# GeoStat-Framework/PyKrige

Hardware: NVIDIA H100
Metric: kriged grid points/sec (N data -> M grid) (higher is better)
Workload: dtype f64

## Files before the change

### pykrige_b200/csrc/api.cu

```cuda
#include <cuda_runtime.h>
#include <string>
#include <vector>
#include <cstring>
#include <cstdio>
#include <cmath>
#include <cstdlib>
#include <algorithm>
#include <thread>
#include <climits>
#include "kernels.h"

#define KB_VERSION 2000
static const int64_t KB_STAGE_PTS = 1 << 20;
#define KB_TILE_COST_32 0.607
#define KB_TILE_COST_16 0.403
static const int64_t KB_STAGE_MIN = 1 << 18;
#define KB_TN_FIELDS 32

struct Src {
    bool grid; int64_t nx, ny, nz;
    const double *a, *b, *c;
    int64_t first, count;
    const double* d_drift; int64_t drift_stride, drift_first;

    Src sub(int64_t o, int64_t m) const {
        Src s = *this; s.first += o; s.count = m; s.drift_first += o; return s;
    }
    PointSource point_source() const {
        PointSource ps{};
        ps.grid = grid ? 1 : 0;
        ps.px = a; ps.py = b; ps.pz = c; ps.gx = a; ps.gy = b; ps.gz = c;
        ps.nx = nx; ps.ny = ny; ps.nz = nz; ps.first = first;
        return ps;
    }
};

enum Tm { TM_ASSEMBLE, TM_CHOLESKY, TM_TRTRI, TM_PACK_DUAL, TM_SOLVE, TM_FINALIZE, TM_H2D, TM_D2H, TM_KNN_SEARCH,
          TM_KNN_SOLVE, TM_SOLVE_LAUNCHES, TM_LAUNCHES, TM_COUNT };
enum Ev { EV_UPLOAD, EV_ADJUSTED, EV_ASM, EV_KNN_BUILT = EV_ASM, EV_FACTOR, EV_INVERT, EV_DUAL, EV_PACKED,
          EV_RUN, EV_RUN_END, EV_H2D, EV_H2D_END, EV_D2H_END, EV_COUNT };

struct DevBuf {
    void* p = nullptr; size_t cap = 0;
    cudaError_t reserve(size_t bytes) {
        if (bytes <= cap) return cudaSuccess;
        if (p) cudaFree(p);
        p = nullptr; cap = 0;
        cudaError_t e = cudaMalloc(&p, bytes);
        if (e == cudaSuccess) cap = bytes;
        return e;
    }
    void release() { if (p) cudaFree(p); p = nullptr; cap = 0; }
    template <typename T> T* as() const { return reinterpret_cast<T*>(p); }
};

struct kb200_ctx {
    int device = 0;
    cudaStream_t stream = nullptr;
    bool own_stream = false;
    std::string err;

    bool described = false, ready = false, knn_ready = false;
    bool local_factor = false;
    int slices = 0;
    int gform = 0;
    int geo = 0;
    int pinv = 0;
    int pinv_sweeps = 0, pinv_rank = 0;
    int dim = 2, dtype = KB200_F64, n = 0, n_pad = 0, ld = 0, n_rl = 0, n_hd = 0, K1 = 1, na = 2, nrb = 0;
    VgParams vg{};
    Aniso an{};
    DriftScale ds{};
    PackMap pm{};
    std::vector<double> hx, hy, hz, hval, hdrift;
    double bb_lo[3] = {0, 0, 0}, bb_hi[3] = {0, 0, 0};
    int nf = 0; int64_t nf_n = 0;
    std::vector<double> hfields;
    int aux_cols = KB_MAXAUX;
    int64_t zstride = 0;
    int pin_blocks = 0;

    DevBuf blob;
    size_t off_consts = 0, off_ax = 0, off_ay = 0, off_az = 0, off_tiles = 0, off_rowscale = 0, blob_bytes = 0;

    DevBuf wC, wW, wT, wF, wRaw, wFlag;
    DevBuf wPts, wOut, wDrift, wScratch, wFstage;
    int num_sms = 132;
    DeviceDrift dd{};
    DevBuf wWells, wExt;
    int n_dev = 0;
    void* pin[2] = {nullptr, nullptr};
    cudaStream_t copy_stream = nullptr;
    cudaEvent_t evk[2] = {}, evc[2] = {};
    cudaStream_t hi_stream = nullptr;
    std::vector<cudaEvent_t> fev;
    DevBuf kSorted, kCells, kFields;
    DevBuf wVario;
    DevBuf wLoo;
    DevBuf wLgo, wLgoM;
    DevBuf wPairs;
    DevBuf wTab;
    std::vector<double> htab;
    double tab_dmax = 0.0; int tab_n = 0;
    KnnParams kp{};
    int k_ncells = 0;

    cudaEvent_t ev[EV_COUNT] = {};
    double tm[TM_COUNT] = {};
    long long launches = 0, solve_launches = 0;
};

static int fail(kb200_ctx* h, int code, const std::string& msg) {
    if (h) h->err = msg;
    return code;
}
#define CU(h, expr) do { cudaError_t _e = (expr); if (_e != cudaSuccess) { \
    return fail(h, _e == cudaErrorMemoryAllocation ? KB200_ENOMEM : KB200_ECUDA, \
                std::string(#expr) + ": " + cudaGetErrorString(_e)); } } while (0)

static size_t align_up(size_t v, size_t a) { return (v + a - 1) / a * a; }

static void drop_problem(kb200_ctx* h) {
    h->described = false; h->ready = false; h->knn_ready = false; h->local_factor = false;
}

struct BlobView { double *hdr, *consts, *ax, *ay, *az; char* tiles; double* rowscale; };
static BlobView blob_view(const kb200_ctx* h) {
    char* p = h->blob.as<char>();
    auto at = [p](size_t off) { return reinterpret_cast<double*>(p + off); };
    return {at(0), at(h->off_consts), at(h->off_ax), at(h->off_ay), at(h->off_az), p + h->off_tiles, at(h->off_rowscale)};
}

enum HdrSlot { HDR_MAGIC = 0, HDR_C0 = 1, HDR_SHIFT = 2, HDR_SCALE = HDR_SHIFT + KB200_MAX_DRIFT + 1,
               HDR_GFORM = HDR_SCALE + KB200_MAX_DRIFT + 1, HDR_DOUBLES = 64 };
static_assert(HDR_GFORM == 34 && HDR_GFORM < HDR_DOUBLES, "blob header layout");
static const double KB_MAGIC = 20260922.0;

static void write_header(const kb200_ctx* h, double* hdr) {
    std::fill(hdr, hdr + HDR_DOUBLES, 0.0);
    hdr[HDR_MAGIC] = KB_MAGIC; hdr[HDR_C0] = h->vg.c0; hdr[HDR_GFORM] = (double)h->gform;
    for (int c = 0; c <= KB200_MAX_DRIFT; ++c) { hdr[HDR_SHIFT + c] = h->ds.shift[c]; hdr[HDR_SCALE + c] = h->ds.scale[c]; }
}

static bool read_header(kb200_ctx* h, const double* hdr) {
    if (hdr[HDR_MAGIC] != KB_MAGIC) return false;
    h->vg.c0 = hdr[HDR_C0];
    h->gform = (int)hdr[HDR_GFORM];
    for (int c = 0; c <= KB200_MAX_DRIFT; ++c) { h->ds.shift[c] = hdr[HDR_SHIFT + c]; h->ds.scale[c] = hdr[HDR_SCALE + c]; }
    return true;
}

enum RawCol { RAW_X, RAW_Y, RAW_Z, RAW_V, RAW_DRIFT };
static double* raw_col(const kb200_ctx* h, int c) { return h->wRaw.as<double>() + (size_t)c * h->n; }
static double* kriged_values(const kb200_ctx* h) { return raw_col(h, h->nf ? RAW_DRIFT + h->n_hd : RAW_V); }

enum AuxBlock { AUX_F, AUX_H, AUX_U };
static double* aux_block(const kb200_ctx* h, int i) {
    return h->wF.as<double>() + (size_t)i * h->aux_cols * h->n_pad;
}

extern "C" int kb200_version(void) { return KB_VERSION; }

extern "C" int kb200_create(kb200_handle* out, int device) {
    if (!out) return KB200_EBADARG;
    *out = nullptr;
    int cnt = 0;
    cudaError_t e = cudaGetDeviceCount(&cnt);
    if (e != cudaSuccess || cnt == 0) return KB200_ECUDA;
    kb200_ctx* h = new kb200_ctx();
    if (device < 0) { if (cudaGetDevice(&device) != cudaSuccess) device = 0; }
    if (device >= cnt) { delete h; return KB200_EBADARG; }
    h->device = device;
    if (cudaSetDevice(device) != cudaSuccess) { delete h; return KB200_ECUDA; }
    if (cudaStreamCreateWithFlags(&h->stream, cudaStreamNonBlocking) != cudaSuccess) { delete h; return KB200_ECUDA; }
    h->own_stream = true;
    for (auto& ev : h->ev) if (cudaEventCreate(&ev) != cudaSuccess) { delete h; return KB200_ECUDA; }
    if (kbk_factor_init() != cudaSuccess || kbk_solve_init() != cudaSuccess || kbk_solve_tf32_init() != cudaSuccess ||
        kbk_solve_i8_init() != cudaSuccess || kbk_ev_init() != cudaSuccess || kbk_pinv_init() != cudaSuccess) { delete h; return KB200_ECUDA; }
    if (cudaDeviceGetAttribute(&h->num_sms, cudaDevAttrMultiProcessorCount, device) != cudaSuccess || h->num_sms < 1) h->num_sms = 132;
    *out = h;
    return KB200_OK;
}

extern "C" void kb200_destroy(kb200_handle h) {
    if (!h) return;
    cudaSetDevice(h->device);
    cudaStreamSynchronize(h->stream);
    for (DevBuf* b : {&h->blob, &h->wC, &h->wW, &h->wT, &h->wF, &h->wRaw, &h->wFlag,
                      &h->wPts, &h->wOut, &h->wDrift, &h->wScratch, &h->wFstage, &h->kSorted, &h->kCells, &h->kFields, &h->wVario, &h->wTab,
                      &h->wLoo, &h->wLgo, &h->wLgoM, &h->wPairs, &h->wWells, &h->wExt}) b->release();
    for (int i = 0; i < 2; ++i) {
        if (h->pin[i]) cudaFreeHost(h->pin[i]);
        if (h->evk[i]) cudaEventDestroy(h->evk[i]);
        if (h->evc[i]) cudaEventDestroy(h->evc[i]);
    }
    if (h->copy_stream) cudaStreamDestroy(h->copy_stream);
    if (h->hi_stream) cudaStreamDestroy(h->hi_stream);
    for (auto& e : h->fev) cudaEventDestroy(e);
    for (auto& ev : h->ev) if (ev) cudaEventDestroy(ev);
    if (h->own_stream && h->stream) cudaStreamDestroy(h->stream);
    delete h;
}

extern "C" const char* kb200_last_error(kb200_handle h) { return h ? h->err.c_str() : "null handle"; }

extern "C" int kb200_set_stream(kb200_handle h, void* s) {
    if (!h) return KB200_EBADARG;
    if (h->own_stream && h->stream) { cudaStreamSynchronize(h->stream); cudaStreamDestroy(h->stream); }
    h->stream = reinterpret_cast<cudaStream_t>(s);
    h->own_stream = false;
    return KB200_OK;
}

extern "C" int kb200_set_coordinates(kb200_handle h, int coordinates_type) {
    if (!h) return KB200_EBADARG;
    if (coordinates_type != KB200_EUCLIDEAN && coordinates_type != KB200_GEOGRAPHIC)
        return fail(h, KB200_EBADARG, "coordinates_type must be KB200_EUCLIDEAN or KB200_GEOGRAPHIC");
    h->geo = coordinates_type == KB200_GEOGRAPHIC ? 1 : 0;
    drop_problem(h);
    return KB200_OK;
}

extern "C" int kb200_set_pseudo_inverse(kb200_handle h, int enable) {
    if (!h) return KB200_EBADARG;
    h->pinv = enable ? 1 : 0;
    drop_problem(h);
    return KB200_OK;
}

extern "C" int kb200_set_values(kb200_handle h, int n_fields, int64_t n, const double* values) {
    if (!h) return KB200_EBADARG;
    drop_problem(h);
    h->nf = 0; h->nf_n = 0; h->hfields.clear();
    if (n_fields == 0) return KB200_OK;
    if (n_fields < 0 || n_fields > KB200_MAX_FIELDS)
        return fail(h, KB200_EBADARG, "n_fields must be in [0, " + std::to_string(KB200_MAX_FIELDS) + "]");
    if (n < 1 || n > (1LL << 30) || !values) return fail(h, KB200_EBADARG, "values: n >= 1 rows and a non-NULL array");
    const size_t cnt = (size_t)n * n_fields;
    for (size_t i = 0; i < cnt; ++i)
        if (!std::isfinite(values[i]))
            return fail(h, KB200_EBADARG, "values must be finite (field " + std::to_string(i / n) + ", row " +
                        std::to_string(i % n) + ")");
    h->hfields.assign(values, values + cnt);
    h->nf = n_fields; h->nf_n = n;
    return KB200_OK;
}

extern "C" void kb200_reset_counters(kb200_handle h) {
    if (!h) return;
    h->launches = 0; h->solve_launches = 0;
    for (double& t : h->tm) t = 0.0;
}

extern "C" int kb200_last_timings(kb200_handle h, double* ms, int n) {
    if (!h || !ms) return KB200_EBADARG;
    h->tm[TM_SOLVE_LAUNCHES] = (double)h->solve_launches;
    h->tm[TM_LAUNCHES] = (double)h->launches;
    int m = std::min(n, (int)TM_COUNT);
    for (int i = 0; i < m; ++i) ms[i] = h->tm[i];
    return m;
}

static double host_gamma(const kb200_ctx* h, const VgParams& v, double d) {
    switch (v.model) {
        case KB200_VG_LINEAR: return v.p0 * d + v.p1;
        case KB200_VG_POWER: return v.p0 * std::pow(d, v.p1) + v.p2;
        case KB200_VG_TABLE: {
            if (h->tab_n < 2) return 1.0;
            const double inv_h = (h->tab_n - 1) / std::sqrt(h->tab_dmax);
            int last = (int)std::min<double>(h->tab_n - 1, std::ceil(std::sqrt(std::max(d, 0.0)) * inv_h));
            double g = h->htab[0];
            for (int i = 0; i <= last; ++i) g = std::max(g, h->htab[2 * (size_t)i]);
            return g;
        }
        default: return v.p0 + v.p2;
    }
}

extern "C" int kb200_set_variogram_table(kb200_handle h, int64_t n_nodes, double dmax, const double* gamma_nodes) {
    if (!h) return KB200_EBADARG;
    if (n_nodes < 16 || n_nodes > (1LL << 26) || !gamma_nodes || !(dmax > 0.0) || !std::isfinite(dmax))
        return fail(h, KB200_EBADARG, "variogram table: 16 <= n_nodes <= 2^26, dmax > 0");
    const int n = (int)n_nodes;
    for (int i = 0; i < n; ++i)
        if (!std::isfinite(gamma_nodes[i])) return fail(h, KB200_EBADARG, "variogram table: the callable must be finite on [0, dmax] (node " + std::to_string(i) + ")");
    drop_problem(h);
    h->htab.resize(2 * (size_t)n);
    for (int i = 0; i < n; ++i) {
        double m;
        if (i == 0) m = -1.5 * gamma_nodes[0] + 2.0 * gamma_nodes[1] - 0.5 * gamma_nodes[2];
        else if (i == n - 1) m = 1.5 * gamma_nodes[n - 1] - 2.0 * gamma_nodes[n - 2] + 0.5 * gamma_nodes[n - 3];
        else m = 0.5 * (gamma_nodes[i + 1] - gamma_nodes[i - 1]);
        h->htab[2 * (size_t)i] = gamma_nodes[i];
        h->htab[2 * (size_t)i + 1] = m;
    }
    h->tab_n = n; h->tab_dmax = dmax;
    cudaSetDevice(h->device);
    CU(h, h->wTab.reserve(h->htab.size() * sizeof(double)));
    CU(h, cudaMemcpyAsync(h->wTab.p, h->htab.data(), h->htab.size() * sizeof(double), cudaMemcpyHostToDevice, h->stream));
    CU(h, cudaStreamSynchronize(h->stream));
    return KB200_OK;
}

static int describe(kb200_ctx* h, bool knn_only, int dim, int dtype, int64_t n,
                    const double* x, const double* y, const double* z, const double* values,
                    const double* center, const double* aniso, int model, const double* vparams, int n_vparams,
                    int exact_values, double eps, int n_rl, int n_hd, const double* drift_data) {
    if (!h) return KB200_EBADARG;
    drop_problem(h);
    if (dim != 2 && dim != 3) return fail(h, KB200_EBADARG, "dim must be 2 or 3");
    if (h->geo && dim != 2) return fail(h, KB200_EBADARG, "geographic coordinates are two-dimensional (lon, lat)");
    if (h->geo && (n_rl || n_hd)) return fail(h, KB200_EUNSUPPORTED, "universal kriging has no geographic mode (uk.py:337)");
    if (dtype < KB200_F64 || dtype > KB200_F64X4)
        return fail(h, KB200_EBADARG, "dtype must be KB200_F64, KB200_F32, KB200_F64X, KB200_F64X5 or KB200_F64X4");
    if (n < 1 || (!knn_only && n > (int64_t)(KB_MAXRB - 1) * KB_BM) || n > (1LL << 30)) return fail(h, KB200_EBADARG, "n out of range");
    if (!x || !y || (dim == 3 && !z) || !values || !center || !aniso || (!vparams && model != KB200_VG_TABLE))
        return fail(h, KB200_EBADARG, "null input array");
    if (model < KB200_VG_LINEAR || model > KB200_VG_TABLE)
// ... 1292 lines not shown
```

### pykrige_b200/csrc/common.cuh

```cuda
#pragma once
#include <cuda_runtime.h>
#include <stdint.h>
#include <math.h>
#include "../../include/krige_b200.h"

#define KB_WARP 32

#define KB_BM 256
#define KB_TN 64
#define KB_BK 16
#define KB_NB 64
#define KB_MAXAUX (KB200_MAX_DRIFT + 2)
#define KB_MAXRB 128

struct VgParams {
    int model;
    double p0, p1, p2;
    double inv_a;
    double c0;
    double eps;
    int exact;
    const double2* tab;
    double tab_inv_h;
    int tab_n;
};

struct Aniso {
    double m[9];
    double c[3];
};

#define KB_GEO 4
#define KB_HASZ(DIM) ((DIM) >= 3)

template <int DIM>
__device__ __forceinline__ void kb_adjust(const Aniso& a, double x, double y, double z,
                                          double& ox, double& oy, double& oz) {
    if (DIM == KB_GEO) {
        const double rad = 0.017453292519943295;
        double slon, clon, slat, clat;
        sincos(x * rad, &slon, &clon);
        sincos(y * rad, &slat, &clat);
        ox = clon * clat; oy = slon * clat; oz = slat;
        return;
    }
    double dx = __dsub_rn(x, a.c[0]);
    double dy = __dsub_rn(y, a.c[1]);
    if (DIM == 2) {
        double rx = __dadd_rn(__dmul_rn(a.m[0], dx), __dmul_rn(a.m[1], dy));
        double ry = __dadd_rn(__dmul_rn(a.m[2], dx), __dmul_rn(a.m[3], dy));
        ox = __dadd_rn(rx, a.c[0]);
        oy = __dadd_rn(ry, a.c[1]);
        oz = 0.0;
    } else {
        double dz = __dsub_rn(z, a.c[2]);
        double rx = __dadd_rn(__dadd_rn(__dmul_rn(a.m[0], dx), __dmul_rn(a.m[1], dy)), __dmul_rn(a.m[2], dz));
        double ry = __dadd_rn(__dadd_rn(__dmul_rn(a.m[3], dx), __dmul_rn(a.m[4], dy)), __dmul_rn(a.m[5], dz));
        double rz = __dadd_rn(__dadd_rn(__dmul_rn(a.m[6], dx), __dmul_rn(a.m[7], dy)), __dmul_rn(a.m[8], dz));
        ox = __dadd_rn(rx, a.c[0]);
        oy = __dadd_rn(ry, a.c[1]);
        oz = __dadd_rn(rz, a.c[2]);
    }
}

__device__ __forceinline__ double kb_exp_neg(double x) {
    const double kd = rint(x * 1.4426950408889634);
    double r = fma(kd, -6.93147180369123816490e-01, x);
    r = fma(kd, -1.90821492927058770002e-10, r);
    double p = 1.6059043836821613e-10;
    p = fma(p, r, 2.08767569878681e-09);
    p = fma(p, r, 2.505210838544172e-08);
    p = fma(p, r, 2.755731922398589e-07);
    p = fma(p, r, 2.7557319223985893e-06);
    p = fma(p, r, 2.48015873015873e-05);
    p = fma(p, r, 1.984126984126984e-04);
    p = fma(p, r, 1.388888888888889e-03);
    p = fma(p, r, 8.333333333333333e-03);
    p = fma(p, r, 4.1666666666666664e-02);
    p = fma(p, r, 1.6666666666666666e-01);
    p = fma(p, r, 0.5);
    p = fma(p, r, 1.0);
    p = fma(p, r, 1.0);
    const int k = (int)kd;
    const double v = __hiloint2double(__double2hiint(p) + (k << 20), __double2loint(p));
    return x < -708.0 ? 0.0 : v;
}

template <int MODEL>
__device__ __forceinline__ double kb_gamma(const VgParams& v, double d) {
    if (MODEL == KB200_VG_LINEAR) {
        return v.p0 * d + v.p1;
    } else if (MODEL == KB200_VG_POWER) {
        return v.p0 * pow(d, v.p1) + v.p2;
    } else if (MODEL == KB200_VG_GAUSSIAN) {
        return v.p0 * (1.0 - kb_exp_neg(-(d * d) * v.inv_a)) + v.p2;
    } else if (MODEL == KB200_VG_EXPONENTIAL) {
        return v.p0 * (1.0 - kb_exp_neg(-d * v.inv_a)) + v.p2;
    } else if (MODEL == KB200_VG_SPHERICAL) {
        if (d <= v.p1) {
            double q = d * v.inv_a;
            return v.p0 * (1.5 * q - 0.5 * q * q * q) + v.p2;
        }
        return v.p0 + v.p2;
    } else if (MODEL == KB200_VG_TABLE) {
        const double u = sqrt(d) * v.tab_inv_h;
        int i = (int)u;
        i = i > v.tab_n - 2 ? v.tab_n - 2 : i;
        const double t = u - (double)i;
        const double2 a = __ldg(v.tab + i), b = __ldg(v.tab + i + 1);
        const double t2 = t * t, t3 = t2 * t;
        return (2.0 * t3 - 3.0 * t2 + 1.0) * a.x + (t3 - 2.0 * t2 + t) * a.y
             + (3.0 * t2 - 2.0 * t3) * b.x + (t3 - t2) * b.y;
    } else {
        double q = d * v.inv_a;
        return v.p0 * (1.0 - (1.0 - q) * kb_exp_neg(-q)) + v.p2;
    }
}

template <int MODEL>
__device__ __forceinline__ double kb_cov_rhs(const VgParams& v, double d) {
    if (v.exact && fabs(d) <= v.eps) return v.c0;
    return v.c0 - kb_gamma<MODEL>(v, d);
}

template <int DIM>
__device__ __forceinline__ double kb_dist(double ax, double ay, double az,
                                          double bx, double by, double bz) {
    if (DIM == KB_GEO) {
        double cx = __dsub_rn(__dmul_rn(ay, bz), __dmul_rn(az, by));
        double cy = __dsub_rn(__dmul_rn(az, bx), __dmul_rn(ax, bz));
        double cz = __dsub_rn(__dmul_rn(ax, by), __dmul_rn(ay, bx));
        double s = sqrt(cx * cx + cy * cy + cz * cz);
        double c = ax * bx + ay * by + az * bz;
        return atan2(s, c) * 57.29577951308232;
    }
    double dx = ax - bx, dy = ay - by;
    double s = dx * dx + dy * dy;
    if (DIM == 3) { double dz = az - bz; s += dz * dz; }
    return sqrt(s);
}

struct PointSource {
    int grid;
    const double* px; const double* py; const double* pz;
    const double* gx; const double* gy; const double* gz;
    long long nx, ny, nz;
    long long first;
};

template <int DIM>
__device__ __forceinline__ void kb_load_point_raw(const PointSource& ps, long long p,
                                                  double& rx, double& ry, double& rz) {
    rz = 0.0;
    long long q = p + ps.first;
    if (ps.grid) {
        long long ix = q % ps.nx;
        long long r = q / ps.nx;
        long long iy = r % ps.ny;
        rx = ps.gx[ix];
        ry = ps.gy[iy];
        if (DIM == 3) { long long iz = r / ps.ny; rz = ps.gz[iz]; }
    } else {
        rx = ps.px[q];
        ry = ps.py[q];
        if (DIM == 3) rz = ps.pz[q];
    }
}

template <int DIM>
__device__ __forceinline__ void kb_load_point(const PointSource& ps, const Aniso& an, long long p,
                                              double& x, double& y, double& z) {
    double rx, ry, rz;
    kb_load_point_raw<DIM>(ps, p, rx, ry, rz);
    kb_adjust<DIM>(an, rx, ry, rz, x, y, z);
}

__device__ __forceinline__ void kb_dmma(double& c0, double& c1, double a, double b) {
    asm volatile("mma.sync.aligned.m8n8k4.row.col.f64.f64.f64.f64 {%0,%1}, {%2}, {%3}, {%0,%1};\n"
                 : "+d"(c0), "+d"(c1) : "d"(a), "d"(b));
}

__device__ __forceinline__ void kb_dmma_16x8x4(double* c, const double* a, double b) {
    asm volatile("mma.sync.aligned.m16n8k4.row.col.f64.f64.f64.f64 {%0,%1,%2,%3}, {%4,%5}, {%6}, {%0,%1,%2,%3};\n"
                 : "+d"(c[0]), "+d"(c[1]), "+d"(c[2]), "+d"(c[3])
                 : "d"(a[0]), "d"(a[1]), "d"(b));
}


__device__ __forceinline__ uint32_t kb_smem_u32(const void* p) { return (uint32_t)__cvta_generic_to_shared(p); }
__device__ __forceinline__ void kb_mbar_init(uint64_t* bar, int count) {
    asm volatile("mbarrier.init.shared::cta.b64 [%0], %1;\n" :: "r"(kb_smem_u32(bar)), "r"(count));
}
__device__ __forceinline__ void kb_fence_mbar_init() {
    asm volatile("fence.mbarrier_init.release.cluster;\n" ::: "memory");
    asm volatile("fence.proxy.async.shared::cta;\n" ::: "memory");
}
__device__ __forceinline__ void kb_mbar_expect_tx(uint64_t* bar, uint32_t bytes) {
    asm volatile("mbarrier.arrive.expect_tx.shared::cta.b64 _, [%0], %1;\n" :: "r"(kb_smem_u32(bar)), "r"(bytes) : "memory");
}
__device__ __forceinline__ void kb_mbar_arrive(uint64_t* bar) {
    asm volatile("mbarrier.arrive.shared::cta.b64 _, [%0];\n" :: "r"(kb_smem_u32(bar)) : "memory");
}
__device__ __forceinline__ bool kb_mbar_try_wait(uint64_t* bar, uint32_t parity) {
    uint32_t ok;
    asm volatile("{\n\t.reg .pred p;\n\t"
                 "mbarrier.try_wait.parity.shared::cta.b64 p, [%1], %2;\n\t"
                 "selp.u32 %0, 1, 0, p;\n\t}\n"
                 : "=r"(ok) : "r"(kb_smem_u32(bar)), "r"(parity) : "memory");
    return ok != 0;
}
__device__ __forceinline__ void kb_mbar_wait(uint64_t* bar, uint32_t parity) {
    for (uint32_t it = 0; it < (1u << 26); ++it)
        if (kb_mbar_try_wait(bar, parity)) return;
    __trap();
}
__device__ __forceinline__ void kb_fence_publish_async() {
    __threadfence();
    asm volatile("fence.proxy.async.global;\n" ::: "memory");
}
__device__ __forceinline__ void kb_bulk_g2s(void* dst, const void* src, uint32_t bytes, uint64_t* bar) {
    asm volatile("cp.async.bulk.shared::cluster.global.mbarrier::complete_tx::bytes [%0], [%1], %2, [%3];\n"
                 :: "r"(kb_smem_u32(dst)), "l"(src), "r"(bytes), "r"(kb_smem_u32(bar)) : "memory");
}

__device__ __forceinline__ uint64_t kb_policy_evict_last() {
    uint64_t p;
    asm volatile("createpolicy.fractional.L2::evict_last.b64 %0, 1.0;\n" : "=l"(p));
    return p;
}
__device__ __forceinline__ uint64_t kb_policy_evict_first() {
    uint64_t p;
    asm volatile("createpolicy.fractional.L2::evict_first.b64 %0, 1.0;\n" : "=l"(p));
    return p;
}
__device__ __forceinline__ void kb_bulk_g2s_hint(void* dst, const void* src, uint32_t bytes, uint64_t* bar, uint64_t policy) {
    asm volatile("cp.async.bulk.shared::cluster.global.mbarrier::complete_tx::bytes.L2::cache_hint [%0], [%1], %2, [%3], %4;\n"
                 :: "r"(kb_smem_u32(dst)), "l"(src), "r"(bytes), "r"(kb_smem_u32(bar)), "l"(policy) : "memory");
}

__device__ __forceinline__ uint64_t kb_wgmma_desc(uint32_t smem_addr, uint32_t lbo, uint32_t sbo) {
    return (uint64_t)((smem_addr >> 4) & 0x3fffu) | ((uint64_t)((lbo >> 4) & 0x3fffu) << 16) |
           ((uint64_t)((sbo >> 4) & 0x3fffu) << 32);
}
__device__ __forceinline__ void kb_wgmma_fence() { asm volatile("wgmma.fence.sync.aligned;\n" ::: "memory"); }
__device__ __forceinline__ void kb_wgmma_commit() { asm volatile("wgmma.commit_group.sync.aligned;\n" ::: "memory"); }
template <int N>
__device__ __forceinline__ void kb_wgmma_wait() { asm volatile("wgmma.wait_group.sync.aligned %0;\n" :: "n"(N) : "memory"); }
__device__ __forceinline__ void kb_reg_fence(float& r) { asm volatile("" : "+f"(r) :: "memory"); }
__device__ __forceinline__ void kb_reg_fence(uint32_t& r) { asm volatile("" : "+r"(r) :: "memory"); }
__device__ __forceinline__ void kb_named_sync(int id, int threads) {
    asm volatile("bar.sync %0, %1;\n" :: "r"(id), "r"(threads) : "memory");
}

#define KB_CUDA_OK(expr) do { cudaError_t _e = (expr); if (_e != cudaSuccess) return _e; } while (0)
```

### pykrige_b200/csrc/solve.cu

```cuda
#include "common.cuh"
#include "kernels.h"

#define PT_STAGES 5
#define PT_THREADS 384
#define PT_CONS0 (PT_THREADS / 32 - 8)
#define PT_STAGE_BYTES ((KB_BM * KB_BK + KB_BK * KB_TN) * 8)

template <int C>
__device__ __forceinline__ void pt_reduce_scatter_step(double* v, int lane, int mask) {
    if constexpr (C >= 2) {
        const bool up = (lane & mask) != 0;
#pragma unroll
        for (int h = 0; h < C / 2; ++h) {
            const double send = up ? v[h] : v[h + C / 2];
            const double keep = up ? v[h + C / 2] : v[h];
            v[h] = keep + __shfl_xor_sync(0xffffffffu, send, mask);
        }
    } else {
        v[0] += __shfl_xor_sync(0xffffffffu, v[0], mask);
    }
}
template <int CNT>
__device__ __forceinline__ void pt_reduce_scatter(double* v, int lane) {
    pt_reduce_scatter_step<CNT>(v, lane, 16);
    pt_reduce_scatter_step<(CNT >= 2 ? CNT / 2 : 1)>(v, lane, 8);
    pt_reduce_scatter_step<(CNT >= 4 ? CNT / 4 : 1)>(v, lane, 4);
}
template <int CNT>
__device__ __forceinline__ int pt_reduce_scatter_index(int i, int lane) {
    int o = i, c = CNT;
    for (int mask = 16; mask >= 4; mask >>= 1) {
        if (c >= 2) { c /= 2; if (lane & mask) o += c; }
        else if (lane & mask) return -1;
    }
    return o;
}

template <int DIM, int MODEL, int NT, bool FIELDS>
__global__ void __launch_bounds__(PT_THREADS, 1) solve_kernel_pt(const __grid_constant__ SolvePtParams P) {
    constexpr int TN = NT * 8;
    extern __shared__ __align__(128) unsigned char smem_raw[];
    double* Ts = reinterpret_cast<double*>(smem_raw);
    double* Bs = Ts + PT_STAGES * KB_BM * KB_BK;
    double* qred = Bs + PT_STAGES * KB_BK * TN;
    double* auxs = qred + 8 * TN;
    uint64_t* full = reinterpret_cast<uint64_t*>(auxs + KB_MAXAUX * TN);
    uint64_t* empty = full + PT_STAGES;

    const int tid = threadIdx.x, lane = tid & 31, warp = tid >> 5;
    const int nk = (P.n + KB_BK - 1) / KB_BK;
    double* scratch = P.scratch + (size_t)blockIdx.x * nk * (KB_BK * TN);
    const double* gt = reinterpret_cast<const double*>(P.tiles);
    const long long ntiles = (P.m + TN - 1) / TN;

    if (tid == 0) {
        for (int s = 0; s < PT_STAGES; ++s) { kb_mbar_init(&full[s], 1); kb_mbar_init(&empty[s], 8); }
        kb_fence_mbar_init();
    }
    __syncthreads();

    const uint32_t stages_per_tile = (uint32_t)(P.pm.tile_off[P.nrb - 1] + P.pm.ktiles[P.nrb - 1]);
    const int cw = warp - PT_CONS0;

    for (uint32_t it = 0; blockIdx.x + (long long)it * gridDim.x < ntiles; ++it) {
        const long long tile = blockIdx.x + (long long)it * gridDim.x;
        const uint32_t git = it * stages_per_tile;
        {
            const int pl = tid % TN;
            const int ks = tid / TN;
            const long long pj = tile * TN + pl;
            const bool pvalid = pj < P.m;
            double px = 0.0, py = 0.0, pz = 0.0;
            if (pvalid) kb_load_point<DIM>(P.ps, P.an, pj, px, py, pz);
            for (int t = ks; t < nk; t += PT_THREADS / TN) {
                double* bt = scratch + (size_t)t * (KB_BK * TN);
#pragma unroll
                for (int k4 = 0; k4 < 4; ++k4) {
                    double v[4];
#pragma unroll
                    for (int kk = 0; kk < 4; ++kk) {
                        const int k = t * KB_BK + k4 * 4 + kk;
                        double val = 0.0;
                        if (pvalid && k < P.n) {
                            double d = kb_dist<DIM>(__ldg(P.ax + k), __ldg(P.ay + k), KB_HASZ(DIM) ? __ldg(P.az + k) : 0.0,
                                                    px, py, pz);
                            val = kb_cov_rhs<MODEL>(P.vg, d);
                        }
                        v[kk] = val;
                    }
                    double2* dst = reinterpret_cast<double2*>(bt + (k4 * NT + (pl >> 3)) * 32 + (pl & 7) * 4);
                    dst[0] = make_double2(v[0], v[1]);
                    dst[1] = make_double2(v[2], v[3]);
                }
            }
            kb_fence_publish_async();
        }
        __syncthreads();

        if (warp == 0) {
            if (lane == 0) {
                uint32_t g = git;
                const uint64_t pol_w = kb_policy_evict_last(), pol_c = kb_policy_evict_first();
                long long tau = 0;
                for (int I = 0; I < P.nrb; ++I) {
                    const int kt = P.pm.ktiles[I];
                    for (int t = 0; t < kt; ++t, ++tau, ++g) {
                        const int s = g % PT_STAGES;
                        kb_mbar_wait(&empty[s], (uint32_t)(((g / PT_STAGES) & 1) ^ 1));
                        kb_mbar_expect_tx(&full[s], (KB_BM * KB_BK + KB_BK * TN) * 8);
                        kb_bulk_g2s_hint(Ts + (size_t)s * KB_BM * KB_BK, gt + (size_t)tau * (KB_BM * KB_BK),
                                         KB_BM * KB_BK * 8, &full[s], pol_w);
                        kb_bulk_g2s_hint(Bs + (size_t)s * KB_BK * TN, scratch + (size_t)t * (KB_BK * TN),
                                         KB_BK * TN * 8, &full[s], pol_c);
                    }
                }
            }
        } else if (warp >= PT_CONS0) {
            uint32_t g = git;
            constexpr int QV = NT >= 4 ? NT / 4 : 1;
            double* qrow = qred + cw * TN;
#pragma unroll
            for (int v = 0; v < QV; ++v) {
                const int o = pt_reduce_scatter_index<2 * NT>(v, lane);
                if (o >= 0) qrow[(o >> 1) * 8 + 2 * (lane & 3) + (o & 1)] = 0.0;
            }
            const int mtl[2] = {cw, 15 - cw};
            for (int I = 0; I < P.nrb; ++I) {
                const uint32_t gend = g + (uint32_t)P.pm.ktiles[I];
                uint32_t glim[2];
#pragma unroll
                for (int q = 0; q < 2; ++q) {
                    const int r0 = I * KB_BM + mtl[q] * 16;
                    if (r0 + 15 >= P.n && r0 < P.n + P.na) glim[q] = gend;
                    else if (r0 >= P.n + P.na) glim[q] = g;
                    else glim[q] = g + (uint32_t)(r0 / KB_BK + 1);
                }
                double acc[2][NT][4];
#pragma unroll
                for (int a = 0; a < 2; ++a)
#pragma unroll
                    for (int b = 0; b < NT; ++b)
#pragma unroll
                        for (int i = 0; i < 4; ++i) acc[a][b][i] = 0.0;
                for (; g < gend; ++g) {
                    const int s = g % PT_STAGES;
                    kb_mbar_wait(&full[s], (uint32_t)((g / PT_STAGES) & 1));
                    const bool on0 = g < glim[0], on1 = g < glim[1];
                    if (on0 || on1) {
                        const double2* ts = reinterpret_cast<const double2*>(Ts + (size_t)s * KB_BM * KB_BK);
                        const double* bs = Bs + (size_t)s * KB_BK * TN;
#pragma unroll
                        for (int k4 = 0; k4 < 4; ++k4) {
                            double fa[2][2];
#pragma unroll
                            for (int q = 0; q < 2; ++q) {
                                const double2 v = ts[(mtl[q] * 4 + k4) * 32 + lane];
                                fa[q][0] = v.x; fa[q][1] = v.y;
                            }
#pragma unroll
                            for (int nt = 0; nt < NT; ++nt) {
                                const double fb = bs[(k4 * NT + nt) * 32 + lane];
                                if (on0) kb_dmma_16x8x4(acc[0][nt], fa[0], fb);
                                if (on1) kb_dmma_16x8x4(acc[1][nt], fa[1], fb);
                            }
                        }
                    }
                    __syncwarp();
                    if (lane == 0) kb_mbar_arrive(&empty[s]);
                }
#pragma unroll
                for (int q = 0; q < 2; ++q)
#pragma unroll
                    for (int h = 0; h < 2; ++h) {
                        const int r = I * KB_BM + mtl[q] * 16 + 8 * h + (lane >> 2);
                        if (r < P.n) {
                            if (!P.gform) {
#pragma unroll
                                for (int nt = 0; nt < NT; ++nt)
#pragma unroll
                                    for (int i = 0; i < 2; ++i) acc[q][nt][2 * h + i] *= acc[q][nt][2 * h + i];
                            } else {
                                const double* bt = P.scratch + ((size_t)blockIdx.x * nk + (r >> 4)) * (KB_BK * TN) +
                                                   ((r & 15) >> 2) * (NT * 32) + (r & 3);
#pragma unroll
                                for (int nt = 0; nt < NT; ++nt)
#pragma unroll
                                    for (int i = 0; i < 2; ++i) {
                                        const int c = nt * 8 + 2 * (lane & 3) + i;
                                        acc[q][nt][2 * h + i] *= bt[(c >> 3) * 32 + (c & 7) * 4];
                                    }
                            }
                        } else {
                            if (r < P.n + P.na) {
                                double* ao = (FIELDS ? P.fstage + (int)(blockIdx.x * P.na * TN) : auxs) + (r - P.n) * TN +
                                             2 * (lane & 3);
#pragma unroll
                                for (int nt = 0; nt < NT; ++nt) {
                                    ao[nt * 8] = acc[q][nt][2 * h];
                                    ao[nt * 8 + 1] = acc[q][nt][2 * h + 1];
                                }
                            }
#pragma unroll
                            for (int nt = 0; nt < NT; ++nt) { acc[q][nt][2 * h] = 0.0; acc[q][nt][2 * h + 1] = 0.0; }
                        }
                    }
                double part[2 * NT];
#pragma unroll
                for (int nt = 0; nt < NT; ++nt)
#pragma unroll
                    for (int i = 0; i < 2; ++i)
                        part[2 * nt + i] = ((acc[0][nt][i] + acc[0][nt][2 + i]) + acc[1][nt][i]) + acc[1][nt][2 + i];
                pt_reduce_scatter<2 * NT>(part, lane);
#pragma unroll
                for (int v = 0; v < QV; ++v) {
                    const int o = pt_reduce_scatter_index<2 * NT>(v, lane);
                    if (o >= 0) qrow[(o >> 1) * 8 + 2 * (lane & 3) + (o & 1)] += part[v];
                }
            }
        }
        __syncthreads();

        if (tid < TN) {
            const long long pj = tile * TN + tid;
            if (pj < P.m) {
                double q = 0.0;
#pragma unroll
                for (int w = 0; w < 8; ++w) q += qred[w * TN + tid];
                if constexpr (FIELDS)
                    kb_finalize_point<DIM, double, true>(P, pj, q, P.fstage + (int)(blockIdx.x * P.na * TN) + tid, TN);
                else
                    kb_finalize_point<DIM, double>(P, pj, q, auxs + tid, TN);
            }
        }
        __syncthreads();
    }
}

static size_t solve_smem_pt() {
    return (size_t)PT_STAGES * (KB_BM * KB_BK + KB_BK * KB_TN) * sizeof(double) + 8 * KB_TN * sizeof(double) +
           KB_MAXAUX * KB_TN * sizeof(double) + 2 * PT_STAGES * sizeof(uint64_t) + 64;
}
size_t kbk_solve_pt_scratch_doubles(int n, int grid) {
    return (size_t)grid * ((n + KB_BK - 1) / KB_BK) * (KB_BK * KB_TN);
}


using PtWidths = KbList<16, 32, 64>;

cudaError_t kbk_solve_init() {
    const int sm = (int)solve_smem_pt();
    return KbDims::for_each([&](auto D) {
        return KbModels::for_each([&](auto M) {
            return PtWidths::for_each([&](auto TN) {
                KB_CUDA_OK(cudaFuncSetAttribute(solve_kernel_pt<D, M, TN / 8, false>,
                                                cudaFuncAttributeMaxDynamicSharedMemorySize, sm));
                if constexpr (TN == 64) return cudaSuccess;
                else return cudaFuncSetAttribute(solve_kernel_pt<D, M, TN / 8, true>,
                                                 cudaFuncAttributeMaxDynamicSharedMemorySize, sm);
            });
        });
    });
}

cudaError_t kbk_solve_pt(int dim, const SolvePtParams& p, int grid, int tile_points, cudaStream_t st) {
    const size_t sm = solve_smem_pt();
    return KbDims::dispatch(dim, [&](auto D) {
        return KbModels::dispatch(p.vg.model, [&](auto M) {
            return PtWidths::dispatch(tile_points, [&](auto TN) {
                if (!p.nf) solve_kernel_pt<D, M, TN / 8, false><<<grid, PT_THREADS, sm, st>>>(p);
                else if constexpr (TN == 64) return cudaErrorInvalidValue;
                else solve_kernel_pt<D, M, TN / 8, true><<<grid, PT_THREADS, sm, st>>>(p);
                return cudaGetLastError();
            });
        });
    });
}
```

Before: 1.774 million.

## Use m16n8k16 FP64 MMA with register-rebalanced warp-specialized producers and consumers

Replaces the per-k4 m16n8k4 DMMA loop with one m16n8k16 FP64 MMA per stage and N-tile. Fragments for all four k4 slices are loaded up front, and stage loops are split into templated variants so the per-stage on0/on1 branches are resolved at compile time. The producer warps now lower their register budget with setmaxnreg and only issue tile loads. The consumer warps raise their budget and also take over the right-hand-side covariance generation and finalization. The tile-cost constants used to choose the tile width are retuned, and the change risks fragment-layout mismatches and barrier-count mismatches between the two warp roles.

Result: faster. 1.927 million, median of 6 (+8.6%).

```diff
diff --git a/pykrige_b200/csrc/api.cu b/pykrige_b200/csrc/api.cu
--- a/pykrige_b200/csrc/api.cu
+++ b/pykrige_b200/csrc/api.cu
@@ -12,8 +12,8 @@
 
 #define KB_VERSION 2000
 static const int64_t KB_STAGE_PTS = 1 << 20;
-#define KB_TILE_COST_32 0.607
-#define KB_TILE_COST_16 0.403
+#define KB_TILE_COST_32 0.534
+#define KB_TILE_COST_16 0.432
 static const int64_t KB_STAGE_MIN = 1 << 18;
 #define KB_TN_FIELDS 32
 
diff --git a/pykrige_b200/csrc/common.cuh b/pykrige_b200/csrc/common.cuh
--- a/pykrige_b200/csrc/common.cuh
+++ b/pykrige_b200/csrc/common.cuh
@@ -180,12 +180,19 @@
                  : "+d"(c0), "+d"(c1) : "d"(a), "d"(b));
 }
 
-__device__ __forceinline__ void kb_dmma_16x8x4(double* c, const double* a, double b) {
-    asm volatile("mma.sync.aligned.m16n8k4.row.col.f64.f64.f64.f64 {%0,%1,%2,%3}, {%4,%5}, {%6}, {%0,%1,%2,%3};\n"
+__device__ __forceinline__ void kb_dmma_16x8x16(double* c, const double* a, const double* b) {
+    asm volatile("mma.sync.aligned.m16n8k16.row.col.f64.f64.f64.f64 {%0,%1,%2,%3}, {%4,%5,%6,%7,%8,%9,%10,%11}, "
+                 "{%12,%13,%14,%15}, {%0,%1,%2,%3};\n"
                  : "+d"(c[0]), "+d"(c[1]), "+d"(c[2]), "+d"(c[3])
-                 : "d"(a[0]), "d"(a[1]), "d"(b));
-}
-
+                 : "d"(a[0]), "d"(a[1]), "d"(a[2]), "d"(a[3]), "d"(a[4]), "d"(a[5]), "d"(a[6]), "d"(a[7]),
+                   "d"(b[0]), "d"(b[1]), "d"(b[2]), "d"(b[3]));
+}
+
+
+template <int R>
+__device__ __forceinline__ void kb_setmaxnreg_inc() { asm volatile("setmaxnreg.inc.sync.aligned.u32 %0;\n" :: "n"(R)); }
+template <int R>
+__device__ __forceinline__ void kb_setmaxnreg_dec() { asm volatile("setmaxnreg.dec.sync.aligned.u32 %0;\n" :: "n"(R)); }
 
 __device__ __forceinline__ uint32_t kb_smem_u32(const void* p) { return (uint32_t)__cvta_generic_to_shared(p); }
 __device__ __forceinline__ void kb_mbar_init(uint64_t* bar, int count) {
diff --git a/pykrige_b200/csrc/solve.cu b/pykrige_b200/csrc/solve.cu
--- a/pykrige_b200/csrc/solve.cu
+++ b/pykrige_b200/csrc/solve.cu
@@ -5,6 +5,8 @@
 #define PT_THREADS 384
 #define PT_CONS0 (PT_THREADS / 32 - 8)
 #define PT_STAGE_BYTES ((KB_BM * KB_BK + KB_BK * KB_TN) * 8)
+#define PT_REGS_PRODUCER 56
+#define PT_REGS_CONSUMER 224
 
 template <int C>
 __device__ __forceinline__ void pt_reduce_scatter_step(double* v, int lane, int mask) {
@@ -34,6 +36,38 @@
         else if (lane & mask) return -1;
     }
     return o;
+}
+
+template <int NT, int ON>
+__device__ __forceinline__ void pt_stages(uint32_t& g, uint32_t gto, double (&acc)[2][NT][4], const double* Ts,
+                                          const double* Bs, uint64_t* full, uint64_t* empty, const int (&mt)[2], int lane) {
+    for (; g < gto; ++g) {
+        const int s = g % PT_STAGES;
+        kb_mbar_wait(&full[s], (uint32_t)((g / PT_STAGES) & 1));
+        if constexpr (ON != 0) {
+            const double2* ts = reinterpret_cast<const double2*>(Ts + (size_t)s * KB_BM * KB_BK);
+            const double* bs = Bs + (size_t)s * KB_BK * NT * 8;
+            double fa[2][8];
+#pragma unroll
+            for (int q = 0; q < 2; ++q)
+                if (ON >> q & 1)
+#pragma unroll
+                    for (int k4 = 0; k4 < 4; ++k4) {
+                        const double2 v = ts[(mt[q] * 4 + k4) * 32 + lane];
+                        fa[q][2 * k4] = v.x; fa[q][2 * k4 + 1] = v.y;
+                    }
+#pragma unroll
+            for (int nt = 0; nt < NT; ++nt) {
+                double fb[4];
+#pragma unroll
+                for (int k4 = 0; k4 < 4; ++k4) fb[k4] = bs[(k4 * NT + nt) * 32 + lane];
+                if (ON & 1) kb_dmma_16x8x16(acc[0][nt], fa[0], fb);
+                if (ON & 2) kb_dmma_16x8x16(acc[1][nt], fa[1], fb);
+            }
+        }
+        __syncwarp();
+        if (lane == 0) kb_mbar_arrive(&empty[s]);
+    }
 }
 
 template <int DIM, int MODEL, int NT, bool FIELDS>
@@ -60,45 +94,46 @@
     __syncthreads();
 
     const uint32_t stages_per_tile = (uint32_t)(P.pm.tile_off[P.nrb - 1] + P.pm.ktiles[P.nrb - 1]);
-    const int cw = warp - PT_CONS0;
-
-    for (uint32_t it = 0; blockIdx.x + (long long)it * gridDim.x < ntiles; ++it) {
-        const long long tile = blockIdx.x + (long long)it * gridDim.x;
-        const uint32_t git = it * stages_per_tile;
-        {
-            const int pl = tid % TN;
-            const int ks = tid / TN;
-            const long long pj = tile * TN + pl;
-            const bool pvalid = pj < P.m;
-            double px = 0.0, py = 0.0, pz = 0.0;
-            if (pvalid) kb_load_point<DIM>(P.ps, P.an, pj, px, py, pz);
-            for (int t = ks; t < nk; t += PT_THREADS / TN) {
-                double* bt = scratch + (size_t)t * (KB_BK * TN);
-#pragma unroll
-                for (int k4 = 0; k4 < 4; ++k4) {
-                    double v[4];
-#pragma unroll
-                    for (int kk = 0; kk < 4; ++kk) {
-                        const int k = t * KB_BK + k4 * 4 + kk;
-                        double val = 0.0;
-                        if (pvalid && k < P.n) {
-                            double d = kb_dist<DIM>(__ldg(P.ax + k), __ldg(P.ay + k), KB_HASZ(DIM) ? __ldg(P.az + k) : 0.0,
-                                                    px, py, pz);
-                            val = kb_cov_rhs<MODEL>(P.vg, d);
-                        }
-                        v[kk] = val;
+    const int cw = __shfl_sync(0xffffffffu, warp - PT_CONS0, 0);
+
+    auto phase_g = [&](long long tile) {
+        const int ct = tid - PT_CONS0 * 32;
+        const int pl = ct % TN;
+        const int ks = ct / TN;
+        const long long pj = tile * TN + pl;
+        const bool pvalid = pj < P.m;
+        double px = 0.0, py = 0.0, pz = 0.0;
+        if (pvalid) kb_load_point<DIM>(P.ps, P.an, pj, px, py, pz);
+        for (int t = ks; t < nk; t += (PT_THREADS - PT_CONS0 * 32) / TN) {
+            double* bt = scratch + (size_t)t * (KB_BK * TN);
+#pragma unroll
+            for (int k4 = 0; k4 < 4; ++k4) {
+                double v[4];
+#pragma unroll
+                for (int kk = 0; kk < 4; ++kk) {
+                    const int k = t * KB_BK + k4 * 4 + kk;
+                    double val = 0.0;
+                    if (pvalid && k < P.n) {
+                        double d = kb_dist<DIM>(__ldg(P.ax + k), __ldg(P.ay + k), KB_HASZ(DIM) ? __ldg(P.az + k) : 0.0,
+                                                px, py, pz);
+                        val = kb_cov_rhs<MODEL>(P.vg, d);
                     }
-                    double2* dst = reinterpret_cast<double2*>(bt + (k4 * NT + (pl >> 3)) * 32 + (pl & 7) * 4);
-                    dst[0] = make_double2(v[0], v[1]);
-                    dst[1] = make_double2(v[2], v[3]);
-                }
-            }
-            kb_fence_publish_async();
-        }
-        __syncthreads();
-
-        if (warp == 0) {
-            if (lane == 0) {
+                    v[kk] = val;
+                }
+                double2* dst = reinterpret_cast<double2*>(bt + (k4 * NT + (pl >> 3)) * 32 + (pl & 7) * 4);
+                dst[0] = make_double2(v[0], v[1]);
+                dst[1] = make_double2(v[2], v[3]);
+            }
+        }
+        kb_fence_publish_async();
+    };
+
+    if (warp < PT_CONS0) {
+        kb_setmaxnreg_dec<PT_REGS_PRODUCER>();
+        for (uint32_t it = 0; blockIdx.x + (long long)it * gridDim.x < ntiles; ++it) {
+            __syncthreads();
+            const uint32_t git = it * stages_per_tile;
+            if (warp == 0 && lane == 0) {
                 uint32_t g = git;
                 const uint64_t pol_w = kb_policy_evict_last(), pol_c = kb_policy_evict_first();
                 long long tau = 0;
@@ -115,7 +150,16 @@
                     }
                 }
             }
-        } else if (warp >= PT_CONS0) {
+            __syncthreads();
+            __syncthreads();
+        }
+    } else {
+        kb_setmaxnreg_inc<PT_REGS_CONSUMER>();
+        for (uint32_t it = 0; blockIdx.x + (long long)it * gridDim.x < ntiles; ++it) {
+            const long long tile = blockIdx.x + (long long)it * gridDim.x;
+            phase_g(tile);
+            __syncthreads();
+            const uint32_t git = it * stages_per_tile;
             uint32_t g = git;
             constexpr int QV = NT >= 4 ? NT / 4 : 1;
             double* qrow = qred + cw * TN;
@@ -142,32 +186,11 @@
                     for (int b = 0; b < NT; ++b)
 #pragma unroll
                         for (int i = 0; i < 4; ++i) acc[a][b][i] = 0.0;
-                for (; g < gend; ++g) {
-                    const int s = g % PT_STAGES;
-                    kb_mbar_wait(&full[s], (uint32_t)((g / PT_STAGES) & 1));
-                    const bool on0 = g < glim[0], on1 = g < glim[1];
-                    if (on0 || on1) {
-                        const double2* ts = reinterpret_cast<const double2*>(Ts + (size_t)s * KB_BM * KB_BK);
-                        const double* bs = Bs + (size_t)s * KB_BK * TN;
-#pragma unroll
-                        for (int k4 = 0; k4 < 4; ++k4) {
-                            double fa[2][2];
-#pragma unroll
-                            for (int q = 0; q < 2; ++q) {
-                                const double2 v = ts[(mtl[q] * 4 + k4) * 32 + lane];
-                                fa[q][0] = v.x; fa[q][1] = v.y;
-                            }
-#pragma unroll
-                            for (int nt = 0; nt < NT; ++nt) {
-                                const double fb = bs[(k4 * NT + nt) * 32 + lane];
-                                if (on0) kb_dmma_16x8x4(acc[0][nt], fa[0], fb);
-                                if (on1) kb_dmma_16x8x4(acc[1][nt], fa[1], fb);
-                            }
-                        }
-                    }
-                    __syncwarp();
-                    if (lane == 0) kb_mbar_arrive(&empty[s]);
-                }
+                const uint32_t glo = min(min(glim[0], glim[1]), gend), ghi = min(max(glim[0], glim[1]), gend);
+                pt_stages<NT, 3>(g, glo, acc, Ts, Bs, full, empty, mtl, lane);
+                if (glim[0] > glim[1]) pt_stages<NT, 1>(g, ghi, acc, Ts, Bs, full, empty, mtl, lane);
+                else pt_stages<NT, 2>(g, ghi, acc, Ts, Bs, full, empty, mtl, lane);
+                pt_stages<NT, 0>(g, gend, acc, Ts, Bs, full, empty, mtl, lane);
 #pragma unroll
                 for (int q = 0; q < 2; ++q)
 #pragma unroll
@@ -217,22 +240,23 @@
                     if (o >= 0) qrow[(o >> 1) * 8 + 2 * (lane & 3) + (o & 1)] += part[v];
                 }
             }
-        }
-        __syncthreads();
-
-        if (tid < TN) {
-            const long long pj = tile * TN + tid;
-            if (pj < P.m) {
-                double q = 0.0;
-#pragma unroll
-                for (int w = 0; w < 8; ++w) q += qred[w * TN + tid];
-                if constexpr (FIELDS)
-                    kb_finalize_point<DIM, double, true>(P, pj, q, P.fstage + (int)(blockIdx.x * P.na * TN) + tid, TN);
-                else
-                    kb_finalize_point<DIM, double>(P, pj, q, auxs + tid, TN);
-            }
-        }
-        __syncthreads();
+            __syncthreads();
+
+            const int ft = tid - PT_CONS0 * 32;
+            if (ft < TN) {
+                const long long pj = tile * TN + ft;
+                if (pj < P.m) {
+                    double q = 0.0;
+#pragma unroll
+                    for (int w = 0; w < 8; ++w) q += qred[w * TN + ft];
+                    if constexpr (FIELDS)
+                        kb_finalize_point<DIM, double, true>(P, pj, q, P.fstage + (int)(blockIdx.x * P.na * TN) + ft, TN);
+                    else
+                        kb_finalize_point<DIM, double>(P, pj, q, auxs + ft, TN);
+                }
+            }
+            __syncthreads();
+        }
     }
 }
 
```
